# Chain123/RecGURU

Measured on AMD Instinct MI355X. Metric: user-sequences/sec (AE+GAN step), higher is better.
Workload: dtype bf16; 1 GPU; cross-domain RecGURU AE+GAN phase-2 iteration (5 critic + 1 generator update), two 100000-item domains; per_gpu_batch=4096, seq_len=200, d_model=128, n_head=4, n_blocks=3, d_ff=512, n_negs=30, user_lengths=U{5..220}, parallelism=dp1

## Files before the change

include/recguru_hip.h:

```cpp
#ifndef RECGURU_HIP_H
#define RECGURU_HIP_H
#include <stddef.h>
#include <stdint.h>
#ifdef __cplusplus
extern "C" {
#endif

#define RG_F32 0
#define RG_BF16 1
#define RG_X3 2

#define RG_ERR_INVALID (-1)
#define RG_ERR_UNSUPPORTED (-2)
#define RG_ERR_HIP (-3)

const char* rg_last_error(void);
int rg_version(void);

int rg_det_enabled(void);
int rg_det_set_arenas(void* fbase0, void* sbase0, unsigned long long bytes0, int bits0,
                      void* fbase1, void* sbase1, unsigned long long bytes1, int bits1);
int rg_det_fault(int clear);

#define RG_PRO_NONE 0
// ... 53 lines not shown


typedef struct {
  const void* qkv;
  const int64_t* key_ids; int64_t pad_value; int causal;
  void* ctx; float* lse;
  int B, L, H, dk;
  float scale;
  float drop_p; unsigned long long seed;
  const float* rowmask;
  const void* x; const void* wqkv; const float* bqkv; int d;
  int x_masked;
  const int* first_live;
  int qkv_hm;
  const void* pad_rows;
} rg_attn_args;
int rg_attn_fwd(const rg_attn_args* args , int dtype, void* stream);
int rg_attn_fwd_x_supported(int d, int dtype, float drop_p);

typedef struct {
  const void* qkv; const void* dctx; const void* ctx; const float* lse;
  const int64_t* key_ids; int64_t pad_value; int causal;
  void* dqkv;
  int B, L, H, dk;
  float scale;
  float drop_p; unsigned long long seed;
  const float* rowmask;
  const float* bqkv; int x_masked;
  const int* first_live;
  int qkv_hm;
} rg_attn_bwd_args;
int rg_attn_bwd(const rg_attn_bwd_args* args , int dtype, void* stream);

int rg_embed_pe_fwd(const void* table, const float* pe, const int64_t* ids, const float* mask, void* out,
                    long long ntok, int L, int d, float drop_p, unsigned long long seed, int dtype, void* stream);
int rg_embed_pe_fwd_rows(const void* table, long long table_rows, const float* pe, const int64_t* ids, const float* mask, void* out,
                         long long ntok, int L, int d, float drop_p, unsigned long long seed, int dtype, void* stream);
int rg_embed_pe_fwd2(const void* table, const float* pe, const int64_t* ids, const float* mask, void* out, void* out2,
                     long long ntok, int L, int d, float drop_p, unsigned long long seed, int dtype, void* stream);
int rg_embed_pe_fwd_split(const float* table_f32, const float* pe, const int64_t* ids, const float* mask, void* out,
                          void* out_lo, long long ntok, int L, int d, float drop_p, unsigned long long seed, void* stream);
int rg_embed_scatter_bwd(const void* dx, const int64_t* ids, const float* mask, float* dE, long long ntok, int d,
                         long long skip_row, float drop_p, unsigned long long seed, int dtype, void* stream);
size_t rg_embed_scatter_binned_workspace(long long ntok, int d, long long table_rows);
int rg_embed_scatter_bwd_binned(const void* dx, const int64_t* ids, const float* mask, float* dE, long long ntok, int d,
// ... 283 lines not shown
  const void* dy2; const void* y2; const float* rstd_c; const float* cgamma; const float* cbeta;
  const void* y1; const float* rstd1; const float* gamma1; const float* beta1;
  const float* rowmask;
  const void* Wot;
  void* dy1; void* dz; void* dctx;
  float* dcgamma; float* dcbeta; float* dz_colsum; float* dgamma1; float* dbeta1; float* partials;
  int M, d, P, w_packed;
  const int* live16;
} rg_attn_out_bwd_cross_args;
int rg_attn_out_bwd_cross(const rg_attn_out_bwd_cross_args* args , int dtype, void* stream);
size_t rg_attn_out_bwd_cross_workspace(int M);
int rg_ffn_bwd_data(const rg_ffn_bwd_args* args , int dtype, void* stream);
int rg_ffn_bwd_data_supported(int d, int dff);
int rg_live_tiles(const float* rowmask, long long M, int* list, void* stream);
int rg_first_live(const float* rowmask, int B, int L, int* first, void* stream);

int rg_attn_lastq_fwd(const void* qlast, const void* kv, const int64_t* key_ids, int64_t pad_value, void* ctx,
                      int B, int L, int H, float scale, float drop_p, unsigned long long seed, int dtype, void* stream,
                      const float* bkv, const int* first_live);
int rg_attn_lastq_bwd(const void* qlast, const void* kv, const void* dctx, const int64_t* key_ids, int64_t pad_value,
                      void* dq, void* dkv, int B, int L, int H, float scale, float drop_p, unsigned long long seed,
                      int dtype, void* stream, const float* bkv, const int* first_live);

typedef struct {
  const void* x; const void* qlast; const void* wk; const void* wv;
  const float* bk; const float* bv;
  const int64_t* key_ids; int64_t pad_value;
  const int* first_live;
  void* ctx;
  const void* dctx;
// ... 29 lines not shown
```

recguru_amd/csrc/attention.hip:

```cpp
#include <stdlib.h>
#include <type_traits>
#include "rg_common.hip.h"
#include "../../include/recguru_hip.h"

#define DK 32
#define NEG_FILL (-1e9f)
#define RESIDENT_MAX_L 416
int rg_attn_long_fwd(const rg_attn_args* a, int dtype, void* stream);
int rg_attn_long_bwd(const rg_attn_bwd_args* a, int dtype, void* stream);

template <typename T> struct VStage;
template <> struct VStage<__bf16> {
  static constexpr bool TRANSPOSED = false;
  static __device__ __forceinline__ void frag(Frag<__bf16>& f, const __bf16* V, int ldv, int k0, int dv0, int li, int lg) {
    typedef __attribute__((ext_vector_type(4))) short s16x4;
    typedef __attribute__((address_space(3))) s16x4 lds_s16x4;
    const int q = li >> 2, p = li & 3;
    const __bf16* p0 = V + (k0 + 4 * lg + q) * ldv + dv0 + 4 * p;
    const __bf16* p1 = p0 + 16 * ldv;
    union { s16x4 s; bf16x4_t b; } u0, u1;
    u0.s = __builtin_amdgcn_ds_read_tr16_b64_v4i16((lds_s16x4*)p0);
    u1.s = __builtin_amdgcn_ds_read_tr16_b64_v4i16((lds_s16x4*)p1);
#pragma unroll
    for (int j = 0; j < 4; ++j) { f.v[j] = u0.b[j]; f.v[4 + j] = u1.b[j]; }
// ... 178 lines not shown
  __shared__ __align__(16) E Ks[LPK * LDK * (X3 ? 2 : 1)];
  __shared__ __align__(16) E Vs[VELEMS * (X3 ? 2 : 1)];
  __shared__ __align__(16) float kbias[LPK];
  constexpr int NW = (NKT + 1) / 2;
  __shared__ __align__(16) unsigned int dmask[DM == 1 ? NW * LPK : 4];
  constexpr bool PLUT = DM == 1 && sizeof(E) == 2;
  constexpr bool MSUM = DM == 0 || PLUT;
  __shared__ __align__(8) unsigned int dlut[PLUT ? 32 : 2];
  __shared__ int klo_s;
  __shared__ int zpre_s;
  __shared__ int fix_s;

  const int tid = threadIdx.x, lane = tid & 63, wave = tid >> 6;
  const int li = lane & 15, lg = lane >> 4;
  int b, h;
  if (!rg_head_of_block((int)blockIdx.x, a.B, a.H, b, h)) return;
  const int L = a.L, P = a.H * DK, ld = 3 * P;
  const T* __restrict__ qkv = XIN ? nullptr : reinterpret_cast<const T*>(a.qkv) + (HM ? (size_t)0 : (size_t)b * L * ld);
  const size_t hm_head = ((size_t)b * a.H + h) * L * DK, hm_tensor = (size_t)a.B * a.H * L * DK;
  int first_q = 0, first_hm = 0;
  if (a.rowmask != nullptr && a.first_live) first_q = min(a.first_live[b], L);
  if constexpr (HM) {
    if (a.x_masked == 2) first_hm = first_q;
  }
  const int nkt = (L + 31) / 32 * 2;
  const int nqt = (L + 15) / 16;
  DropCfg drop = make_drop(a.drop_p, a.seed);
  if constexpr (DM == 2) drop.onebit = 0u;
  if (tid == 0) { klo_s = L; zpre_s = L; fix_s = 0; }
  if (PLUT && tid < 16) {
    dlut[2 * tid] = ((tid & 1) ? 0xFFFFu : 0u) | ((tid & 2) ? 0xFFFF0000u : 0u);
// ... 448 lines not shown

template <typename T, int NKT>
__global__ __launch_bounds__(256, 2) void attn_bwd_kernel(rg_attn_bwd_args a) {
  constexpr int LPK = NKT * 16;
  constexpr int LDT = LPK + 8;
  __shared__ __align__(16) T Qt[DK * LDT];
  __shared__ __align__(16) T dOt[DK * LDT];
  T* const Kt = Qt;
  __shared__ float lse_s[LPK];
  __shared__ float dl_s[LPK];
  __shared__ unsigned char kpad[LPK];

  const int tid = threadIdx.x, lane = tid & 63, wave = tid >> 6;
  const int li = lane & 15, lg = lane >> 4;
  int b, h;
  if (!rg_head_of_block((int)blockIdx.x, a.B, a.H, b, h)) return;
  const int L = a.L, P = a.H * DK, ld = 3 * P;
  const T* __restrict__ qkv = reinterpret_cast<const T*>(a.qkv) + (size_t)b * L * ld;
  const T* __restrict__ dO = reinterpret_cast<const T*>(a.dctx) + (size_t)b * L * P + h * DK;
  const T* __restrict__ O = reinterpret_cast<const T*>(a.ctx) + (size_t)b * L * P + h * DK;
  T* __restrict__ dqkv = reinterpret_cast<T*>(a.dqkv) + (size_t)b * L * ld;
  const int nt = (L + 31) / 32 * 2;
  const DropCfg gdrop = make_drop(a.drop_p, a.seed);
  const unsigned int gbase = ((unsigned int)b * a.H + h) * L;
  const unsigned int glp4 = rg_lpad(L);

  for (int c = tid; c < LPK * 4; c += 256) {
    const int row = c >> 2, c8 = (c & 3) * 8;
    float qv[8], gv[8], ov[8];
    if (row < L) {
      load8(qv, qkv + (size_t)row * ld + h * DK + c8);
// ... 164 lines not shown
  T* const Ks = RESTAGE ? QKVG : QKVG + LPK * LDR;
  T* const Vs = RESTAGE ? QKVG + LPK * LDR : QKVG + 2 * LPK * LDR;
  T* const Gs = RESTAGE ? QKVG + LPK * LDR : QKVG + 3 * LPK * LDR;
  __shared__ __align__(16) float lse2_s[LPK];
  __shared__ __align__(16) float dl_s[LPK];
  __shared__ __align__(16) float rowp_s[LPK];
  __shared__ __align__(16) float kbias[LPK];
  constexpr int NW = (NKT + 1) / 2;
  __shared__ __align__(16) unsigned int dmask[DM == 1 ? NW * LPK : 4];
  __shared__ int qlive[NKT];
  __shared__ int klo_s;

  const int tid = threadIdx.x, lane = tid & 63, wave = tid >> 6;
  const int li = lane & 15, lg = lane >> 4;
  int b, h;
  if (!rg_head_of_block((int)blockIdx.x, a.B, a.H, b, h)) return;
  const int L = a.L, P = a.H * DK, ld = 3 * P;
  const size_t hm_tensor = (size_t)a.B * a.H * L * DK;
  const G* __restrict__ qrow = reinterpret_cast<const G*>(a.qkv) + (a.qkv_hm ? ((size_t)b * a.H + h) * L * DK : (size_t)b * L * ld + h * DK);
  const G* __restrict__ krow = qrow + (a.qkv_hm ? hm_tensor : (size_t)P);
  const G* __restrict__ vrow = qrow + (a.qkv_hm ? 2 * hm_tensor : (size_t)(2 * P));
  const int qld = a.qkv_hm ? DK : ld;
  const G* __restrict__ dO = reinterpret_cast<const G*>(a.dctx) + (size_t)b * L * P + h * DK;
  const G* __restrict__ O = reinterpret_cast<const G*>(a.ctx) + (size_t)b * L * P + h * DK;
  G* __restrict__ dqkv = reinterpret_cast<G*>(a.dqkv) + (size_t)b * L * ld;
  const int nt = (L + 31) / 32 * 2;
  const float c2 = a.scale * 1.4426950408889634f;
  DropCfg drop = make_drop(a.drop_p, a.seed);
  if constexpr (DM == 2) drop.onebit = 0u;
  const unsigned int dbase = ((unsigned int)b * a.H + h) * L;
  const unsigned int lp4 = rg_lpad(L);
// ... 627 lines not shown
```

recguru_amd/csrc/elementwise.hip:

```cpp
#include <stdlib.h>
#include "rg_common.hip.h"
#include "rg_det.hip.h"
#include "../../include/recguru_hip.h"

#define EW_BLOCK 256
static inline int ew_grid(long long work_items, int per_block) {
  long long g = (work_items + per_block - 1) / per_block;
  if (g < 1) g = 1;
  if (g > 256LL * 16) g = 256LL * 16;
  return (int)g;
}

template <typename T>
__global__ __launch_bounds__(EW_BLOCK) void embed_pe_fwd_kernel(const T* __restrict__ table, const float* __restrict__ pe,
                                                               const int64_t* __restrict__ ids,
                                                               const float* __restrict__ mask, T* __restrict__ out,
                                                               long long ntok, int L, int d, DropCfg drop) {
  const int cpr = d >> 3;
  const long long total = ntok * cpr;
  for (long long i = (long long)blockIdx.x * EW_BLOCK + threadIdx.x; i < total; i += (long long)gridDim.x * EW_BLOCK) {
    const long long tok = i / cpr;
    const int c8 = (int)(i - tok * cpr) * 8;
    const float m = mask[tok];
    const int64_t id = ids[tok];
// ... 1099 lines not shown
    for (int l0 = 0; l0 < L && f == L; l0 += 64) {
      const int l = l0 + lane;
      const unsigned long long m = __ballot(l < L && rowmask[(size_t)b * L + l] != 0.f);
      if (m) f = l0 + __builtin_ctzll(m);
    }
    if (lane == 0) first[b] = f;
  }
}
extern "C" int rg_first_live(const float* rowmask, int B, int L, int* first, void* stream) {
  if (B <= 0 || L <= 0) return 0;
  hipLaunchKernelGGL(first_live_kernel, dim3(ew_grid((long long)B * 64, EW_BLOCK)), dim3(EW_BLOCK), 0, (hipStream_t)stream, rowmask, B, L, first);
  RG_CHECK_LAUNCH();
  return 0;
}

extern "C" int rg_live_tiles(const float* rowmask, long long M, int* list, void* stream) {
  if (M <= 0) return 0;
  const long long nt = (M + 15) >> 4;
  const int nwords = (int)((nt + 63) >> 6);
  if (nwords > LIVE_MAXW) return rg_set_error_msg(RG_ERR_UNSUPPORTED, "live_tiles: more than 8.4 M rows");
  unsigned long long* masks = reinterpret_cast<unsigned long long*>((reinterpret_cast<uintptr_t>(list + 1 + nt) + 7) & ~(uintptr_t)7);
  hipLaunchKernelGGL(live_flags_kernel, dim3(ew_grid(nt, EW_BLOCK)), dim3(EW_BLOCK), 0, (hipStream_t)stream, rowmask, M, masks);
  const int smem = nwords * 12;
  hipFuncSetAttribute(reinterpret_cast<const void*>(live_compact_kernel), hipFuncAttributeMaxDynamicSharedMemorySize, smem);
  hipLaunchKernelGGL(live_compact_kernel, dim3(1), dim3(1024), smem, (hipStream_t)stream, nt, list, masks);
  RG_CHECK_LAUNCH();
  return 0;
}

__global__ __launch_bounds__(EW_BLOCK) void pad_mask_kernel(const int64_t* __restrict__ ids, int64_t pad, float* __restrict__ out, long long n) {
// ... 491 lines not shown
```

recguru_amd/csrc/rg_common.hip.h:

```cpp
#pragma once
#include <hip/hip_runtime.h>
#include <stdint.h>

typedef __attribute__((ext_vector_type(4))) float f32x4;
typedef __attribute__((ext_vector_type(8))) __bf16 bf16x8_t;
typedef __attribute__((ext_vector_type(4))) __bf16 bf16x4_t;

#define RG_F32 0
#define RG_BF16 1
#define RG_X3 2
#define RG_WAVE 64

struct x3 {
  float f;
  x3() = default;
  __host__ __device__ __forceinline__ x3(float v) : f(v) {}
  __host__ __device__ __forceinline__ operator float() const { return f; }
};
static_assert(sizeof(x3) == 4 && alignof(x3) == 4, "x3 is layout-identical to float");
__device__ __forceinline__ const float* fptr(const x3* p) { return reinterpret_cast<const float*>(p); }
__device__ __forceinline__ float* fptr(x3* p) { return reinterpret_cast<float*>(p); }

template <typename T> struct Frag;
template <> struct Frag<float> { float v[8]; };
// ... 358 lines not shown
    rg_keep4(c, base + 16u, k1);
  }
}
__host__ __device__ inline DropCfg make_drop(float p, unsigned long long seed) {
  DropCfg c;
  unsigned int s = (unsigned int)seed * 0x9E3779B1u ^ ((unsigned int)(seed >> 32) * 0x85EBCA77u + 0x165667B1u);
  s ^= s >> 15; s *= 0x2c1b3c6du; s ^= s >> 12;
  c.seed = s;
  c.thresh = p > 0.f ? (unsigned int)((double)p * 65536.0 + 0.5) : 0u;
  c.inv_keep = p > 0.f ? 1.f / (1.f - p) : 1.f;
  c.onebit = p == 0.5f ? 1u : 0u;
  return c;
}
__host__ __device__ inline unsigned int rg_lpad(int L) { return (unsigned int)((L + 31) & ~31); }

__device__ __forceinline__ bool rg_head_of_block(int bid, int B, int H, int& b, int& h) {
  const int hp = (H + 1) >> 1;
  const int xcd = bid & 7, rnd = bid >> 3;
  const int slot = (rnd >> 1) * 8 + xcd;
  b = slot / hp;
  h = 2 * (slot - b * hp) + (rnd & 1);
  return b < B && h < H;
}
static inline int rg_head_grid(int B, int H) {
  const int slots = B * ((H + 1) >> 1);
  return ((slots + 7) / 8) * 16;
}

__device__ __forceinline__ void lds_barrier() { asm volatile("s_waitcnt lgkmcnt(0)\n\ts_barrier" ::: "memory"); }

struct LiveWalk {
  const int* list;
  int nlive, cap, v, blk;
  int wg, nwg;
  __device__ __forceinline__ void init(const int* live16, int M) { init(live16, M, (int)blockIdx.x, (int)gridDim.x); }
  __device__ __forceinline__ void init(const int* live16, int M, int wg_, int nwg_) {
    wg = wg_;
// ... 48 lines not shown
```

recguru_amd/hip.py:

```python
import ctypes
import os

import torch

_HERE = os.path.dirname(os.path.abspath(__file__))
DETERMINISTIC = os.environ.get("RG_DETERMINISTIC", "0") not in ("", "0")
LIB_PATH = os.environ.get("RG_HIP_LIB") or os.path.join(_HERE, "librecguru_hip_det.so" if DETERMINISTIC else "librecguru_hip.so")
_lib = None

F32, BF16, X3 = 0, 1, 2
SPLIT_OPERANDS = False
PRO_NONE, PRO_GELU = 0, 1
EPI_NONE, EPI_RELU, EPI_MUL_POSMASK, EPI_GELU_GRAD, EPI_ADD, EPI_RESID_LN, EPI_DROP_GELU = 0, 1, 2, 3, 4, 5, 6

c_p, c_i, c_f, c_l = ctypes.c_void_p, ctypes.c_int, ctypes.c_float, ctypes.c_int64
c_u64 = ctypes.c_uint64


class GemmNtArgs(ctypes.Structure):
    _fields_ = [("A", c_p), ("lda", c_i), ("W", c_p), ("ldw", c_i), ("bias", c_p), ("C", c_p), ("ldc", c_i),
                ("c_is_f32", c_i), ("M", c_i), ("N", c_i), ("K", c_i), ("prologue", c_i), ("epilogue", c_i),
                ("aux", c_p), ("ldaux", c_i), ("gamma", c_p), ("beta", c_p), ("rowmask", c_p),
                ("rstd_out", c_p), ("ln_eps", c_f), ("debug_ablate", c_i), ("epi_scale", c_f),
                ("epi_nonzero_scale", c_f), ("drop_p", c_f), ("drop_seed", c_u64), ("live16", c_p),
                ("skip_dead_fill", c_i), ("c_hm_L", c_i), ("C2", c_p), ("w_packed", c_i)]


class GemmTnArgs(ctypes.Structure):
    _fields_ = [("Y", c_p), ("ldy", c_i), ("X", c_p), ("ldx", c_i), ("dW", c_p), ("lddw", c_i), ("colsum", c_p),
                ("T", c_i), ("N1", c_i), ("N2", c_i), ("prologue_x", c_i), ("scale", c_f), ("splits", c_i),
                ("use_tr", c_i), ("live16", c_p), ("partials", c_p), ("colsum_T", c_i)]


class AttnArgs(ctypes.Structure):
    _fields_ = [("qkv", c_p), ("key_ids", c_p), ("pad_value", c_l), ("causal", c_i), ("ctx", c_p), ("lse", c_p),
                ("B", c_i), ("L", c_i), ("H", c_i), ("dk", c_i), ("scale", c_f), ("drop_p", c_f), ("seed", c_u64), ("rowmask", c_p),
                ("x", c_p), ("wqkv", c_p), ("bqkv", c_p), ("d", c_i), ("x_masked", c_i), ("first_live", c_p),
                ("qkv_hm", c_i), ("pad_rows", c_p)]


class AttnBwdArgs(ctypes.Structure):
    _fields_ = [("qkv", c_p), ("dctx", c_p), ("ctx", c_p), ("lse", c_p), ("key_ids", c_p), ("pad_value", c_l),
                ("causal", c_i), ("dqkv", c_p), ("B", c_i), ("L", c_i), ("H", c_i), ("dk", c_i), ("scale", c_f),
                ("drop_p", c_f), ("seed", c_u64), ("rowmask", c_p), ("bqkv", c_p), ("x_masked", c_i), ("first_live", c_p),
                ("qkv_hm", c_i)]


class PostAttnArgs(ctypes.Structure):
    _fields_ = [("ctx", c_p), ("x", c_p), ("Wo", c_p), ("bo", c_p), ("g1", c_p), ("be1", c_p),
                ("o_bcast", c_p), ("gc", c_p), ("bec", c_p), ("L", c_i),
                ("W1", c_p), ("b1", c_p), ("W2", c_p), ("b2", c_p), ("g2", c_p), ("be2", c_p),
                ("rowmask", c_p), ("out", c_p),
                ("y_save", c_p), ("rstd1", c_p), ("y2_save", c_p), ("rstd_c", c_p), ("h1_save", c_p), ("rstd2", c_p),
                ("M", c_i), ("d", c_i), ("P", c_i), ("dff", c_i), ("eps", c_f),
                ("drop_p", c_f), ("seed_h1", c_u64), ("seed_out", c_u64),
                ("cross_s", c_p), ("cross_oh", c_p), ("cross_bo", c_p), ("H", c_i), ("live16", c_p),
                ("skip_dead_saves", c_i), ("w_packed", c_i), ("x_lo", c_p), ("out_lo", c_p)]


class FfnBwdArgs(ctypes.Structure):
# ... 15 lines not shown
                ("y1", c_p), ("rstd1", c_p), ("gamma1", c_p), ("beta1", c_p), ("rowmask", c_p), ("Wot", c_p),
                ("dy1", c_p), ("dz", c_p), ("dctx", c_p),
                ("dcgamma", c_p), ("dcbeta", c_p), ("dz_colsum", c_p), ("dgamma1", c_p), ("dbeta1", c_p), ("partials", c_p),
                ("M", c_i), ("d", c_i), ("P", c_i), ("w_packed", c_i), ("live16", c_p)]


SYMBOLS = ["rg_last_error", "rg_version", "rg_gemm_nt", "rg_gemm_tn", "rg_attn_fwd", "rg_attn_bwd",
           "rg_embed_pe_fwd", "rg_embed_pe_fwd_rows", "rg_embed_scatter_bwd", "rg_ln_bwd", "rg_bcast_add_ln", "rg_seq_sum", "rg_colsum",
           "rg_outer_posmask", "rg_interpolate", "rg_gp_penalty", "rg_sum", "rg_adam", "rg_cast",
           "rg_item_loss_fwd", "rg_item_loss_bwd", "rg_post_attn_fwd",
           "rg_attn_lastq_fwd", "rg_attn_lastq_bwd",
           "rg_cross_drop_scale", "rg_seq_wsum", "rg_gemm_nt_plan", "rg_gemm_tn_plan", "rg_gemm_tn_workspace", "rg_gemm_tn_layer", "rg_gemm_tn_layer_supported", "rg_gemm_tn_layer_workspace", "rg_ln_bwd_workspace", "rg_cast_multi",
           "rg_item_loss_bwd_binned_workspace", "rg_item_loss_bwd_binned", "rg_adam_multi", "rg_rank_scores",
           "rg_assemble_batch", "rg_sample_negatives", "rg_sample_negatives_alias", "rg_dropout", "rg_cross_rows", "rg_live_tiles",
           "rg_adam_multi_dev", "rg_disc_rows", "rg_disc_supported", "rg_attn_fwd_x_supported", "rg_pad_mask", "rg_last_rows",
           "rg_ffn_bwd_data", "rg_ffn_bwd_data_supported", "rg_ffn_bwd_ln_workspace", "rg_first_live",
           "rg_attn_out_bwd", "rg_attn_out_bwd_workspace", "rg_attn_out_bwd_cross", "rg_attn_out_bwd_cross_workspace",
           "rg_item_loss_train_supported", "rg_item_loss_train", "rg_item_loss_scatter_binned", "rg_scale_dev",
           "rg_attn_lastq_x_supported", "rg_attn_lastq_x_fwd", "rg_attn_lastq_x_bwd", "rg_attn_lastq_xf_fwd", "rg_attn_lastq_xf_bwd",
           "rg_embed_scatter_binned_workspace", "rg_embed_scatter_bwd_binned", "rg_embed_pe_fwd_split", "rg_mse",
           "rg_dropout_gelu", "rg_add_drop_ln", "rg_cross_add_ln", "rg_embed_pe_fwd2",
           "rg_det_enabled", "rg_det_set_arenas", "rg_det_fault",
           "rg_full_ce_supported", "rg_full_ce_fwd", "rg_full_ce_dw",
           "rg_shared_ce_supported", "rg_shared_ce_bwd_workspace", "rg_shared_ce_fwd", "rg_shared_ce_bwd",
           "rg_topk_workspace", "rg_topk_scores", "rg_topk_list_workspace", "rg_topk_list",
           "rg_grad_sqnorm_multi", "rg_adam_multi_dev2",
           "rg_pos_grad_workspace", "rg_pos_grad",
           "rg_attn_probs", "rg_attn_cross_probs", "rg_attn_rollout"]
LOSS_SAMPLED_CE, LOSS_BPR, LOSS_BPR_SAS = 0, 1, 2
c_ll = ctypes.c_longlong

# ... 337 lines not shown
    dt = mt_of(next(pr[0] for pr in probs if pr is not None))
    cw = (ctypes.c_int * 4)(*wgs)
    if not lib().rg_gemm_tn_layer_supported(ctypes.byref(args), cw, dt):
        if sc is not None:
            sc.commit()
        return False
    try:
        _check(lib().rg_gemm_tn_layer(ctypes.byref(args), cw, dt, _stream()), "rg_gemm_tn_layer")
    finally:
        if sc is not None:
            sc.commit()
    return True


def attn_fwd(qkv, key_ids, pad_value, causal, H, need_lse=True, drop_p=0.0, seed=0, rowmask=None, x_masked=False, bqkv=None,
             pad_rows=None):
    hm = qkv.dim() == 5
    if hm:
        _, B, Hq, L, dk = qkv.shape
        assert Hq == H and dk == 32 and pad_rows is not None and pad_rows.shape == (3 * H + 1, 32) and pad_rows.dtype == qkv.dtype
        assert qkv.is_contiguous() and key_ids.dtype == torch.int64 and key_ids.is_contiguous()
    else:
        B, L, P3 = qkv.shape
        assert P3 == 3 * H * 32 and qkv.is_contiguous() and key_ids.dtype == torch.int64 and key_ids.is_contiguous()
    ctx = torch.empty(B, L, H * 32, device=qkv.device, dtype=qkv.dtype)
    lse = torch.empty(B, H, L, device=qkv.device, dtype=torch.float32) if need_lse else None
    a = AttnArgs(_p(qkv), _p(key_ids), int(pad_value), int(bool(causal)), _p(ctx), _p(lse), B, L, H, 32,
                 1.0 / (32 ** 0.5), drop_p, seed, _p(rowmask), None, None, _p(bqkv) if x_masked else None, 0,
                 (2 if bqkv is not None else 1) if (x_masked and rowmask is not None) else 0,
                 _p(first_live(rowmask, B, L)) if (x_masked and rowmask is not None and bqkv is not None) else None,
                 1 if hm else 0, _p(pad_rows) if hm else None)
    _check(lib().rg_attn_fwd(ctypes.byref(a), mt_of(qkv), _stream()), "rg_attn_fwd")
    return ctx, lse


def attn_fwd_x_supported(d, dtype, drop_p):
    return bool(lib().rg_attn_fwd_x_supported(int(d), BF16 if dtype == torch.bfloat16 else F32, c_f(drop_p)))


def attn_fwd_x(x, wqkv, bqkv, key_ids, pad_value, causal, H, drop_p=0.0, seed=0, rowmask=None, x_masked=False):
    B, L, d = x.shape
    assert x.is_contiguous() and wqkv.is_contiguous() and wqkv.shape == (3 * H * 32, d) and wqkv.dtype == x.dtype
    assert bqkv.dtype == torch.float32 and bqkv.numel() == 3 * H * 32 and key_ids.dtype == torch.int64 and key_ids.is_contiguous()
    ctx = torch.empty(B, L, H * 32, device=x.device, dtype=x.dtype)
    a = AttnArgs(None, _p(key_ids), int(pad_value), int(bool(causal)), _p(ctx), None, B, L, H, 32,
                 1.0 / (32 ** 0.5), drop_p, seed, _p(rowmask), _p(x), _p(wqkv), _p(bqkv), d, int(bool(x_masked)), None, 0, None)
    _check(lib().rg_attn_fwd(ctypes.byref(a), mt_of(x), _stream()), "rg_attn_fwd")
    return ctx


def attn_bwd(qkv, dctx, ctx, lse, key_ids, pad_value, causal, H, drop_p=0.0, seed=0, rowmask=None, bqkv=None):
    hm = qkv.dim() == 5
    B, L = (qkv.shape[1], qkv.shape[3]) if hm else qkv.shape[:2]
    assert dctx.is_contiguous() and ctx.is_contiguous() and qkv.is_contiguous()
    dqkv = torch.empty(B, L, 3 * H * 32, device=qkv.device, dtype=qkv.dtype)
    sub = bqkv is not None and rowmask is not None
    a = AttnBwdArgs(_p(qkv), _p(dctx), _p(ctx), _p(lse), _p(key_ids), int(pad_value), int(bool(causal)),
                    _p(dqkv), B, L, H, 32, 1.0 / (32 ** 0.5), drop_p, seed, _p(rowmask), _p(bqkv) if sub else None, 2 if sub else 0,
                    _p(first_live(rowmask, B, L)) if sub else None, 1 if hm else 0)
    _check(lib().rg_attn_bwd(ctypes.byref(a), mt_of(qkv), _stream()), "rg_attn_bwd")
    return dqkv


def _vp(t):
    return ctypes.c_void_p(_p(t))


class AttnProbsArgs(ctypes.Structure):
    _fields_ = [("qkv", c_p), ("key_ids", c_p), ("pad_value", c_l), ("causal", c_i), ("probs", c_p), ("b_stride", ctypes.c_longlong),
                ("B", c_i), ("L", c_i), ("H", c_i), ("dk", c_i), ("scale", c_f)]


def _map_dest(out, layer, B, H, L, dev):
    if out is None:
# ... 831 lines not shown


_FIRST = {}


def first_live(rowmask, B, L):
    key = (rowmask.data_ptr(), rowmask._version, B, L)
    hit = _FIRST.get(key)
    if hit is not None:
        return hit[1]
    out = torch.empty(B, device=rowmask.device, dtype=torch.int32)
    _check(lib().rg_first_live(_vp(rowmask), B, L, _vp(out), _stream()), "rg_first_live")
    if len(_FIRST) >= 32:
        _FIRST.pop(next(iter(_FIRST)))
    _FIRST[key] = (rowmask, out)
    return out


def post_attn_fwd(ctx, x, Wo, bo, g1, be1, W1, b1, W2, b2, g2, be2, rowmask, save=False, cross=None, L=0, eps=1e-8,
                  drop_p=0.0, seed_h1=0, seed_out=0, cross_drop=None, compact=True, skip_dead_saves=False, w_packed=False,
                  x_lo=None):
    M, P = ctx.shape
    d = x.shape[1]
    dff = W1.shape[0]
    dev = ctx.device
    live16 = None
    if rowmask is not None and M >= COMPACT_MIN_ROWS and compact:
        live16 = live_tiles(rowmask, M)
    out = torch.empty(M, d, device=dev, dtype=ctx.dtype)
    sv = {}
# ... 399 lines not shown
```

recguru_amd/ops.py:

```python
import os
import weakref

import torch

from . import hip

_COMPUTE = torch.bfloat16
LN_EPS = 1e-8
GP_LAMBDA = 0.1


def set_compute_dtype(dt):
    global _COMPUTE, _MIXED
    _MIXED = dt == "mixed"
    x3 = dt in ("bf16x3", "mixed")
    if x3:
        dt = torch.float32
    elif dt == "bf16":
        dt = torch.bfloat16
    elif dt == "f32":
        dt = torch.float32
    assert dt in (torch.float32, torch.bfloat16)
    _COMPUTE = dt
    hip.SPLIT_OPERANDS = x3
# ... 511 lines not shown
FUSE_ATTN_OUT_BWD = True
FUSE_ATTN_OUT_BWD_CROSS = True
LASTQ_FROM_X = True
LASTQ_FOLD_PREFIX = True
ATTN_RESIDENT_MAX_L = 416


def _zero_rows_live(rowmask, M, x_masked, K=128, N=384):
    if not x_masked or rowmask is None or not _lists_ok() or M < max(hip.COMPACT_MIN_ROWS, 4096):
        return None
    if not ((K == 128 and N in (128, 256, 384, 512)) or (K in (256, 384, 512) and N % 128 == 0 and 128 <= N <= 1024)):
        return None
    return hip.live_tiles(rowmask, M)


def _qkv_attn_fwd(x2, B, L, key_ids, pad_value, causal, H, Wq, bq, Wk, bk, Wv, bv, need_grad, drop_p=0.0, seed=0,
                  rowmask=None, x_masked=False, allow_unwritten=False):
    wqkv = shadow_cat((Wq, Wk, Wv))
    bqkv = bias_cat((bq, bk, bv))
    if not need_grad and FUSE_QKV_INFERENCE and L <= ATTN_RESIDENT_MAX_L and hip.attn_fwd_x_supported(x2.shape[1], _COMPUTE, drop_p):
        ctx_ = hip.attn_fwd_x(x2.view(B, L, -1), wqkv, bqkv, key_ids, pad_value, causal, H, drop_p=drop_p, seed=seed,
                              rowmask=rowmask, x_masked=x_masked and rowmask is not None)
        return None, ctx_, None
    live = _zero_rows_live(rowmask, x2.shape[0], x_masked, x2.shape[1], wqkv.shape[0])
    sub = live is not None and QKV_BIAS_ROWS_IN_ATTENTION and allow_unwritten and _unwritten_qkv_ok() and L <= ATTN_RESIDENT_MAX_L
    if (QKV_HEAD_MAJOR and _COMPUTE == torch.bfloat16 and (H, x2.shape[1]) in ((4, 128), (8, 256)) and x2.shape[0] >= 4096
            and 16 <= L <= ATTN_RESIDENT_MAX_L and (not need_grad or QKV_HEAD_MAJOR_TRAIN)):
        qkv = hip.gemm_nt(x2, wqkv, bqkv, live=live, skip_dead_fill=1 if sub else 2, headmajor_L=L)
        ctx_, lse = hip.attn_fwd(qkv, key_ids, pad_value, causal, H, need_lse=need_grad, drop_p=drop_p, seed=seed, rowmask=rowmask,
                                 x_masked=x_masked, bqkv=bqkv if sub else None, pad_rows=pad_rows_cat((bq, bk, bv), H))
        return qkv, ctx_, lse
    qkv = hip.gemm_nt(x2, wqkv, bqkv, live=live, skip_dead_fill=1 if sub else 2)
    ctx_, lse = hip.attn_fwd(qkv.view(B, L, -1), key_ids, pad_value, causal, H, need_lse=need_grad, drop_p=drop_p, seed=seed,
                             rowmask=rowmask, x_masked=x_masked, bqkv=bqkv if sub else None)
    return qkv, ctx_, lse


def attn_map(x, key_ids, pad_value, causal, H, Wq, bq, Wk, bk, Wv, bv, out=None, layer=None):
    with torch.no_grad():
        B, L, d = x.shape
        x2 = x.detach().contiguous().view(B * L, d)
        qkv = hip.gemm_nt(x2, shadow_cat((Wq, Wk, Wv)), bias_cat((bq, bk, bv)))
        return hip.attn_probs(qkv.view(B, L, -1), key_ids.contiguous(), int(pad_value), H, bool(causal), out=out, layer=layer)


def _attn_block_fwd(x2, B, L, key_ids, pad_value, causal, H, Wq, bq, Wk, bk, Wv, bv, Wo, bo, g, be, need_grad,
                    drop_p=0.0, seed=0, rowmask=None, x_masked=False):
    qkv, ctx_, lse = _qkv_attn_fwd(x2, B, L, key_ids, pad_value, causal, H, Wq, bq, Wk, bk, Wv, bv, need_grad, drop_p, seed,
                                   rowmask, x_masked)
# ... 29 lines not shown
        hip.gemm_tn(dz, ctx_.view(B * L, P), dWo, dbo, live=live if live is not None else _live_tn(rowmask, dz.shape[0], P, d))
        dctx = hip.gemm_nt(dz, shadow(Wo, transpose=True), live=live, skip_dead_fill=True)
    dx, gqkv = _attn_block_bwd_qkv(dz, dctx, live, x2, saved, B, L, key_ids, pad_value, causal, H, prm, drop_p, seed, rowmask, x_masked)
    return dx, gqkv + (rWo, rbo, rg, rbe)


def _attn_block_bwd_qkv(dz, dctx, live, x2, saved, B, L, key_ids, pad_value, causal, H, prm, drop_p=0.0, seed=0, rowmask=None,
                        x_masked=False):
    Wq, bq, Wk, bk, Wv, bv = prm[:6]
    qkv, ctx_, lse, _ = saved
    d = x2.shape[1]
    P = prm[6].shape[1]
    sub = (QKV_BIAS_ROWS_IN_ATTENTION and x_masked == 2 and _unwritten_qkv_ok() and L <= ATTN_RESIDENT_MAX_L
           and _zero_rows_live(rowmask, x2.shape[0], True, d, 3 * P) is not None)
    dqkv = hip.attn_bwd(qkv if qkv.dim() == 5 else qkv.view(B, L, -1), dctx.view(B, L, P), ctx_, lse, key_ids, pad_value, causal, H,
                        drop_p=drop_p, seed=seed, rowmask=rowmask, bqkv=bias_cat((bq, bk, bv)) if sub else None)
    dqkv2 = dqkv.view(B * L, 3 * P)
    (dWqkv, rW), (dbqkv, rb) = _gt_cat((Wq, Wk, Wv)), _gt_cat((bq, bk, bv))
    _tn(dqkv2, x2, dWqkv, dbqkv)
    Wt = shadow_cat((Wq, Wk, Wv), transpose=True)
    if (WS_SPLIT_K_DX and _ws_tier() and dqkv2.shape[0] >= 4096 and 3 * P == 768 and d % 128 == 0
            and 128 < d <= 1024):
        dx = hip.gemm_nt(dqkv2[:, :384], Wt[:, :384], epilogue=hip.EPI_ADD, aux=dz, live=live)
        dx = hip.gemm_nt(dqkv2[:, 384:], Wt[:, 384:], epilogue=hip.EPI_ADD, aux=dx, out=dx, live=live)
    else:
        dx = hip.gemm_nt(dqkv2, Wt, epilogue=hip.EPI_ADD, aux=dz, live=live)
    return dx, (rW[0], rb[0], rW[1], rb[1], rW[2], rb[2])


def _ffn_block_fwd(y, rowmask, W1, b1, W2, b2, g, be, drop_p=0.0, seed_h1=0, seed_out=0):
    M, d = y.shape
# ... 697 lines not shown
```

Baseline: 871,400 user-sequences/sec.

## Schedule attention blocks longest-sequence-first via on-device sequence ordering

```diff
diff --git a/include/recguru_hip.h b/include/recguru_hip.h
--- a/include/recguru_hip.h
+++ b/include/recguru_hip.h
@@ -91,6 +91,7 @@
   const int* first_live;
   int qkv_hm;
   const void* pad_rows;
+  const int* seq_order;
 } rg_attn_args;
 int rg_attn_fwd(const rg_attn_args* args , int dtype, void* stream);
 int rg_attn_fwd_x_supported(int d, int dtype, float drop_p);
@@ -106,6 +107,7 @@
   const float* bqkv; int x_masked;
   const int* first_live;
   int qkv_hm;
+  const int* seq_order;
 } rg_attn_bwd_args;
 int rg_attn_bwd(const rg_attn_bwd_args* args , int dtype, void* stream);
 
@@ -419,6 +421,7 @@
 int rg_ffn_bwd_data_supported(int d, int dff);
 int rg_live_tiles(const float* rowmask, long long M, int* list, void* stream);
 int rg_first_live(const float* rowmask, int B, int L, int* first, void* stream);
+int rg_seq_order(const int* first_live, int B, int L, int* order, void* stream);
 
 int rg_attn_lastq_fwd(const void* qlast, const void* kv, const int64_t* key_ids, int64_t pad_value, void* ctx,
                       int B, int L, int H, float scale, float drop_p, unsigned long long seed, int dtype, void* stream,
diff --git a/recguru_amd/csrc/attention.hip b/recguru_amd/csrc/attention.hip
--- a/recguru_amd/csrc/attention.hip
+++ b/recguru_amd/csrc/attention.hip
@@ -216,7 +216,7 @@
   const int tid = threadIdx.x, lane = tid & 63, wave = tid >> 6;
   const int li = lane & 15, lg = lane >> 4;
   int b, h;
-  if (!rg_head_of_block((int)blockIdx.x, a.B, a.H, b, h)) return;
+  if (!rg_head_of_block((int)blockIdx.x, a.B, a.H, a.seq_order, b, h)) return;
   const int L = a.L, P = a.H * DK, ld = 3 * P;
   const T* __restrict__ qkv = XIN ? nullptr : reinterpret_cast<const T*>(a.qkv) + (HM ? (size_t)0 : (size_t)b * L * ld);
   const size_t hm_head = ((size_t)b * a.H + h) * L * DK, hm_tensor = (size_t)a.B * a.H * L * DK;
@@ -695,7 +695,7 @@
   const int tid = threadIdx.x, lane = tid & 63, wave = tid >> 6;
   const int li = lane & 15, lg = lane >> 4;
   int b, h;
-  if (!rg_head_of_block((int)blockIdx.x, a.B, a.H, b, h)) return;
+  if (!rg_head_of_block((int)blockIdx.x, a.B, a.H, a.seq_order, b, h)) return;
   const int L = a.L, P = a.H * DK, ld = 3 * P;
   const T* __restrict__ qkv = reinterpret_cast<const T*>(a.qkv) + (size_t)b * L * ld;
   const T* __restrict__ dO = reinterpret_cast<const T*>(a.dctx) + (size_t)b * L * P + h * DK;
@@ -890,7 +890,7 @@
   const int tid = threadIdx.x, lane = tid & 63, wave = tid >> 6;
   const int li = lane & 15, lg = lane >> 4;
   int b, h;
-  if (!rg_head_of_block((int)blockIdx.x, a.B, a.H, b, h)) return;
+  if (!rg_head_of_block((int)blockIdx.x, a.B, a.H, a.seq_order, b, h)) return;
   const int L = a.L, P = a.H * DK, ld = 3 * P;
   const size_t hm_tensor = (size_t)a.B * a.H * L * DK;
   const G* __restrict__ qrow = reinterpret_cast<const G*>(a.qkv) + (a.qkv_hm ? ((size_t)b * a.H + h) * L * DK : (size_t)b * L * ld + h * DK);
diff --git a/recguru_amd/csrc/elementwise.hip b/recguru_amd/csrc/elementwise.hip
--- a/recguru_amd/csrc/elementwise.hip
+++ b/recguru_amd/csrc/elementwise.hip
@@ -1137,6 +1137,89 @@
   return 0;
 }
 
+#define SEQ_ORDER_WAVES 16
+#define SO_KR 4
+__global__ __launch_bounds__(SEQ_ORDER_WAVES * 64) void seq_order_kernel(const int* __restrict__ first, int B, int L, int nb, int nbits,
+                                                                         int* __restrict__ order) {
+  extern __shared__ int so_smem[];
+  int* const cnt = so_smem;
+  int* const tot = so_smem + SEQ_ORDER_WAVES * nb;
+  const int tid = threadIdx.x, lane = tid & 63, wave = tid >> 6;
+  const int seg = ((B + SEQ_ORDER_WAVES * 64 - 1) / (SEQ_ORDER_WAVES * 64)) * 64;
+  const int nch = seg >> 6;
+  const int maxt = (L + 15) >> 4;
+  const int lo = wave * seg;
+  const unsigned long long lower = (1ull << lane) - 1ull;
+  int* const mine = cnt + wave * nb;
+  auto chunk_key = [&](int c) {
+    const int i = lo + c * 64 + lane;
+    return i < B ? maxt - ((L - min(max(first[i], 0), L) + 15) >> 4) : -1;
+  };
+  auto same_key = [&](int key) {
+    unsigned long long m = __ballot(key >= 0);
+    for (int bit = 0; bit < nbits; ++bit) {
+      const unsigned long long bal = __ballot((key >> bit) & 1);
+      m &= ((key >> bit) & 1) ? bal : ~bal;
+    }
+    return m;
+  };
+  auto count = [&](int key) {
+    const unsigned long long m = same_key(key);
+    if (key >= 0 && (m & lower) == 0) mine[key] += __popcll(m);
+    __builtin_amdgcn_fence(__ATOMIC_ACQ_REL, "wavefront");
+  };
+  auto place = [&](int key, int c) {
+    const unsigned long long m = same_key(key);
+    const int below = __popcll(m & lower);
+    if (key >= 0) order[tot[key] + mine[key] + below] = lo + c * 64 + lane;
+    if (key >= 0 && below == 0) mine[key] += __popcll(m);
+    __builtin_amdgcn_fence(__ATOMIC_ACQ_REL, "wavefront");
+  };
+  int kreg[SO_KR];
+#pragma unroll
+  for (int c = 0; c < SO_KR; ++c) kreg[c] = c < nch ? chunk_key(c) : -1;
+  for (int i = tid; i < (SEQ_ORDER_WAVES + 1) * nb; i += SEQ_ORDER_WAVES * 64) so_smem[i] = 0;
+  __syncthreads();
+#pragma unroll
+  for (int c = 0; c < SO_KR; ++c)
+    if (c < nch) count(kreg[c]);
+  for (int c = SO_KR; c < nch; ++c) count(chunk_key(c));
+  __syncthreads();
+  for (int k = tid; k < nb; k += SEQ_ORDER_WAVES * 64) {
+    int s = 0;
+    for (int w = 0; w < SEQ_ORDER_WAVES; ++w) { const int c = cnt[w * nb + k]; cnt[w * nb + k] = s; s += c; }
+    tot[k] = s;
+  }
+  __syncthreads();
+  if (wave == 0) {
+    int carry = 0;
+    for (int k0 = 0; k0 < nb; k0 += 64) {
+      const int v = k0 + lane < nb ? tot[k0 + lane] : 0;
+      int inc = v;
+      for (int d = 1; d < 64; d <<= 1) { const int u = __shfl_up(inc, d); if (lane >= d) inc += u; }
+      if (k0 + lane < nb) tot[k0 + lane] = carry + inc - v;
+      carry += __shfl(inc, 63);
+    }
+  }
+  __syncthreads();
+#pragma unroll
+  for (int c = 0; c < SO_KR; ++c)
+    if (c < nch) place(kreg[c], c);
+  for (int c = SO_KR; c < nch; ++c) place(chunk_key(c), c);
+}
+extern "C" int rg_seq_order(const int* first_live, int B, int L, int* order, void* stream) {
+  if (B <= 0) return 0;
+  if (L <= 0 || L > 16384 || !first_live || !order) return rg_set_error_msg(RG_ERR_INVALID, "seq_order: needs first_live, order and 0 < L <= 16384");
+  const int nb = ((L + 15) >> 4) + 1;
+  int nbits = 0;
+  while ((1 << nbits) < nb) ++nbits;
+  const int smem = (SEQ_ORDER_WAVES + 1) * nb * (int)sizeof(int);
+  if (smem > 48 * 1024) hipFuncSetAttribute(reinterpret_cast<const void*>(seq_order_kernel), hipFuncAttributeMaxDynamicSharedMemorySize, smem);
+  hipLaunchKernelGGL(seq_order_kernel, dim3(1), dim3(SEQ_ORDER_WAVES * 64), smem, (hipStream_t)stream, first_live, B, L, nb, nbits, order);
+  RG_CHECK_LAUNCH();
+  return 0;
+}
+
 extern "C" int rg_live_tiles(const float* rowmask, long long M, int* list, void* stream) {
   if (M <= 0) return 0;
   const long long nt = (M + 15) >> 4;
diff --git a/recguru_amd/csrc/rg_common.hip.h b/recguru_amd/csrc/rg_common.hip.h
--- a/recguru_amd/csrc/rg_common.hip.h
+++ b/recguru_amd/csrc/rg_common.hip.h
@@ -396,13 +396,16 @@
 }
 __host__ __device__ inline unsigned int rg_lpad(int L) { return (unsigned int)((L + 31) & ~31); }
 
-__device__ __forceinline__ bool rg_head_of_block(int bid, int B, int H, int& b, int& h) {
+__device__ __forceinline__ bool rg_head_of_block(int bid, int B, int H, const int* __restrict__ seq_order, int& b, int& h) {
   const int hp = (H + 1) >> 1;
   const int xcd = bid & 7, rnd = bid >> 3;
   const int slot = (rnd >> 1) * 8 + xcd;
-  b = slot / hp;
-  h = 2 * (slot - b * hp) + (rnd & 1);
-  return b < B && h < H;
+  const int rank = slot / hp;
+  h = 2 * (slot - rank * hp) + (rnd & 1);
+  b = rank;
+  if (rank >= B || h >= H) return false;
+  if (seq_order) b = seq_order[rank];
+  return true;
 }
 static inline int rg_head_grid(int B, int H) {
   const int slots = B * ((H + 1) >> 1);
diff --git a/recguru_amd/hip.py b/recguru_amd/hip.py
--- a/recguru_amd/hip.py
+++ b/recguru_amd/hip.py
@@ -36,14 +36,14 @@
     _fields_ = [("qkv", c_p), ("key_ids", c_p), ("pad_value", c_l), ("causal", c_i), ("ctx", c_p), ("lse", c_p),
                 ("B", c_i), ("L", c_i), ("H", c_i), ("dk", c_i), ("scale", c_f), ("drop_p", c_f), ("seed", c_u64), ("rowmask", c_p),
                 ("x", c_p), ("wqkv", c_p), ("bqkv", c_p), ("d", c_i), ("x_masked", c_i), ("first_live", c_p),
-                ("qkv_hm", c_i), ("pad_rows", c_p)]
+                ("qkv_hm", c_i), ("pad_rows", c_p), ("seq_order", c_p)]
 
 
 class AttnBwdArgs(ctypes.Structure):
     _fields_ = [("qkv", c_p), ("dctx", c_p), ("ctx", c_p), ("lse", c_p), ("key_ids", c_p), ("pad_value", c_l),
                 ("causal", c_i), ("dqkv", c_p), ("B", c_i), ("L", c_i), ("H", c_i), ("dk", c_i), ("scale", c_f),
                 ("drop_p", c_f), ("seed", c_u64), ("rowmask", c_p), ("bqkv", c_p), ("x_masked", c_i), ("first_live", c_p),
-                ("qkv_hm", c_i)]
+                ("qkv_hm", c_i), ("seq_order", c_p)]
 
 
 class PostAttnArgs(ctypes.Structure):
@@ -89,7 +89,7 @@
            "rg_item_loss_bwd_binned_workspace", "rg_item_loss_bwd_binned", "rg_adam_multi", "rg_rank_scores",
            "rg_assemble_batch", "rg_sample_negatives", "rg_sample_negatives_alias", "rg_dropout", "rg_cross_rows", "rg_live_tiles",
            "rg_adam_multi_dev", "rg_disc_rows", "rg_disc_supported", "rg_attn_fwd_x_supported", "rg_pad_mask", "rg_last_rows",
-           "rg_ffn_bwd_data", "rg_ffn_bwd_data_supported", "rg_ffn_bwd_ln_workspace", "rg_first_live",
+           "rg_ffn_bwd_data", "rg_ffn_bwd_data_supported", "rg_ffn_bwd_ln_workspace", "rg_first_live", "rg_seq_order",
            "rg_attn_out_bwd", "rg_attn_out_bwd_workspace", "rg_attn_out_bwd_cross", "rg_attn_out_bwd_cross_workspace",
            "rg_item_loss_train_supported", "rg_item_loss_train", "rg_item_loss_scatter_binned", "rg_scale_dev",
            "rg_attn_lastq_x_supported", "rg_attn_lastq_x_fwd", "rg_attn_lastq_x_bwd", "rg_attn_lastq_xf_fwd", "rg_attn_lastq_xf_bwd",
@@ -457,7 +457,7 @@
 
 
 def attn_fwd(qkv, key_ids, pad_value, causal, H, need_lse=True, drop_p=0.0, seed=0, rowmask=None, x_masked=False, bqkv=None,
-             pad_rows=None):
+             pad_rows=None, seq_order=None):
     hm = qkv.dim() == 5
     if hm:
         _, B, Hq, L, dk = qkv.shape
@@ -472,27 +472,34 @@
                  1.0 / (32 ** 0.5), drop_p, seed, _p(rowmask), None, None, _p(bqkv) if x_masked else None, 0,
                  (2 if bqkv is not None else 1) if (x_masked and rowmask is not None) else 0,
                  _p(first_live(rowmask, B, L)) if (x_masked and rowmask is not None and bqkv is not None) else None,
-                 1 if hm else 0, _p(pad_rows) if hm else None)
+                 1 if hm else 0, _p(pad_rows) if hm else None, _p(_order_arg(seq_order, B)))
     _check(lib().rg_attn_fwd(ctypes.byref(a), mt_of(qkv), _stream()), "rg_attn_fwd")
     return ctx, lse
 
 
+def _order_arg(seq_order, B):
+    if seq_order is not None:
+        assert seq_order.dtype == torch.int32 and seq_order.is_contiguous() and seq_order.numel() == B
+    return seq_order
+
+
 def attn_fwd_x_supported(d, dtype, drop_p):
     return bool(lib().rg_attn_fwd_x_supported(int(d), BF16 if dtype == torch.bfloat16 else F32, c_f(drop_p)))
 
 
-def attn_fwd_x(x, wqkv, bqkv, key_ids, pad_value, causal, H, drop_p=0.0, seed=0, rowmask=None, x_masked=False):
+def attn_fwd_x(x, wqkv, bqkv, key_ids, pad_value, causal, H, drop_p=0.0, seed=0, rowmask=None, x_masked=False, seq_order=None):
     B, L, d = x.shape
     assert x.is_contiguous() and wqkv.is_contiguous() and wqkv.shape == (3 * H * 32, d) and wqkv.dtype == x.dtype
     assert bqkv.dtype == torch.float32 and bqkv.numel() == 3 * H * 32 and key_ids.dtype == torch.int64 and key_ids.is_contiguous()
     ctx = torch.empty(B, L, H * 32, device=x.device, dtype=x.dtype)
     a = AttnArgs(None, _p(key_ids), int(pad_value), int(bool(causal)), _p(ctx), None, B, L, H, 32,
-                 1.0 / (32 ** 0.5), drop_p, seed, _p(rowmask), _p(x), _p(wqkv), _p(bqkv), d, int(bool(x_masked)), None, 0, None)
+                 1.0 / (32 ** 0.5), drop_p, seed, _p(rowmask), _p(x), _p(wqkv), _p(bqkv), d, int(bool(x_masked)), None, 0, None,
+                 _p(_order_arg(seq_order, B)))
     _check(lib().rg_attn_fwd(ctypes.byref(a), mt_of(x), _stream()), "rg_attn_fwd")
     return ctx
 
 
-def attn_bwd(qkv, dctx, ctx, lse, key_ids, pad_value, causal, H, drop_p=0.0, seed=0, rowmask=None, bqkv=None):
+def attn_bwd(qkv, dctx, ctx, lse, key_ids, pad_value, causal, H, drop_p=0.0, seed=0, rowmask=None, bqkv=None, seq_order=None):
     hm = qkv.dim() == 5
     B, L = (qkv.shape[1], qkv.shape[3]) if hm else qkv.shape[:2]
     assert dctx.is_contiguous() and ctx.is_contiguous() and qkv.is_contiguous()
@@ -500,7 +507,7 @@
     sub = bqkv is not None and rowmask is not None
     a = AttnBwdArgs(_p(qkv), _p(dctx), _p(ctx), _p(lse), _p(key_ids), int(pad_value), int(bool(causal)),
                     _p(dqkv), B, L, H, 32, 1.0 / (32 ** 0.5), drop_p, seed, _p(rowmask), _p(bqkv) if sub else None, 2 if sub else 0,
-                    _p(first_live(rowmask, B, L)) if sub else None, 1 if hm else 0)
+                    _p(first_live(rowmask, B, L)) if sub else None, 1 if hm else 0, _p(_order_arg(seq_order, B)))
     _check(lib().rg_attn_bwd(ctypes.byref(a), mt_of(qkv), _stream()), "rg_attn_bwd")
     return dqkv
 
@@ -1362,6 +1369,22 @@
     if len(_FIRST) >= 32:
         _FIRST.pop(next(iter(_FIRST)))
     _FIRST[key] = (rowmask, out)
+    return out
+
+
+_ORDER = {}
+
+
+def seq_order(rowmask, B, L):
+    key = (rowmask.data_ptr(), rowmask._version, B, L)
+    hit = _ORDER.get(key)
+    if hit is not None:
+        return hit[1]
+    out = torch.empty(B, device=rowmask.device, dtype=torch.int32)
+    _check(lib().rg_seq_order(_vp(first_live(rowmask, B, L)), B, L, _vp(out), _stream()), "rg_seq_order")
+    if len(_ORDER) >= 32:
+        _ORDER.pop(next(iter(_ORDER)))
+    _ORDER[key] = (rowmask, out)
     return out
 
 
diff --git a/recguru_amd/ops.py b/recguru_amd/ops.py
--- a/recguru_amd/ops.py
+++ b/recguru_amd/ops.py
@@ -549,6 +549,12 @@
     return hip.live_tiles(rowmask, M)
 
 
+def _seq_order(rowmask, B, L, H):
+    if rowmask is None or L > ATTN_RESIDENT_MAX_L or B * H <= 512 or rowmask.numel() != B * L:
+        return None
+    return hip.seq_order(rowmask, B, L)
+
+
 def _qkv_attn_fwd(x2, B, L, key_ids, pad_value, causal, H, Wq, bq, Wk, bk, Wv, bv, need_grad, drop_p=0.0, seed=0,
                   rowmask=None, x_masked=False, allow_unwritten=False):
     wqkv = shadow_cat((Wq, Wk, Wv))
@@ -559,15 +565,17 @@
         return None, ctx_, None
     live = _zero_rows_live(rowmask, x2.shape[0], x_masked, x2.shape[1], wqkv.shape[0])
     sub = live is not None and QKV_BIAS_ROWS_IN_ATTENTION and allow_unwritten and _unwritten_qkv_ok() and L <= ATTN_RESIDENT_MAX_L
+    order = _seq_order(rowmask, B, L, H) if (need_grad and causal) else None
     if (QKV_HEAD_MAJOR and _COMPUTE == torch.bfloat16 and (H, x2.shape[1]) in ((4, 128), (8, 256)) and x2.shape[0] >= 4096
             and 16 <= L <= ATTN_RESIDENT_MAX_L and (not need_grad or QKV_HEAD_MAJOR_TRAIN)):
         qkv = hip.gemm_nt(x2, wqkv, bqkv, live=live, skip_dead_fill=1 if sub else 2, headmajor_L=L)
         ctx_, lse = hip.attn_fwd(qkv, key_ids, pad_value, causal, H, need_lse=need_grad, drop_p=drop_p, seed=seed, rowmask=rowmask,
-                                 x_masked=x_masked, bqkv=bqkv if sub else None, pad_rows=pad_rows_cat((bq, bk, bv), H))
+                                 x_masked=x_masked, bqkv=bqkv if sub else None, pad_rows=pad_rows_cat((bq, bk, bv), H),
+                                 seq_order=order)
         return qkv, ctx_, lse
     qkv = hip.gemm_nt(x2, wqkv, bqkv, live=live, skip_dead_fill=1 if sub else 2)
     ctx_, lse = hip.attn_fwd(qkv.view(B, L, -1), key_ids, pad_value, causal, H, need_lse=need_grad, drop_p=drop_p, seed=seed,
-                             rowmask=rowmask, x_masked=x_masked, bqkv=bqkv if sub else None)
+                             rowmask=rowmask, x_masked=x_masked, bqkv=bqkv if sub else None, seq_order=order)
     return qkv, ctx_, lse
 
 
@@ -627,7 +635,8 @@
     sub = (QKV_BIAS_ROWS_IN_ATTENTION and x_masked == 2 and _unwritten_qkv_ok() and L <= ATTN_RESIDENT_MAX_L
            and _zero_rows_live(rowmask, x2.shape[0], True, d, 3 * P) is not None)
     dqkv = hip.attn_bwd(qkv if qkv.dim() == 5 else qkv.view(B, L, -1), dctx.view(B, L, P), ctx_, lse, key_ids, pad_value, causal, H,
-                        drop_p=drop_p, seed=seed, rowmask=rowmask, bqkv=bias_cat((bq, bk, bv)) if sub else None)
+                        drop_p=drop_p, seed=seed, rowmask=rowmask, bqkv=bias_cat((bq, bk, bv)) if sub else None,
+                        seq_order=_seq_order(rowmask, B, L, H))
     dqkv2 = dqkv.view(B * L, 3 * P)
     (dWqkv, rW), (dbqkv, rb) = _gt_cat((Wq, Wk, Wv)), _gt_cat((bq, bk, bv))
     _tn(dqkv2, x2, dWqkv, dbqkv)
```

Result: no change. 874,500 user-sequences/sec, median of 6 (+0.3%).
